# duylebkHCM/doc2tex

Hardware: AMD Instinct MI355X
Metric: formulas/s (greedy decode, 128x512 crops) (higher is better)
Workload: dtype bf16x3

## Files before the change

doc2tex_amd/_lib.py:

```python
import ctypes as C
import os

_HERE = os.path.dirname(os.path.abspath(__file__))
LIB_PATH = os.path.join(_HERE, "csrc", "libd2t.so")
if os.environ.get("D2T_PROBE_LIB"):
    LIB_PATH = os.path.abspath(os.environ["D2T_PROBE_LIB"])

D2T_OK = 0
D2T_EINVAL, D2T_ENOMEM, D2T_EHIP, D2T_ESTATE = 1, 2, 3, 4
ENC_RESNET, ENC_HYBRID_VIT, ENC_VGG_BILSTM, ENC_RESNET_BILSTM, ENC_VGG = 0, 1, 2, 3, 4
DEC_TFM, DEC_ATTN = 0, 1
ATTN_KEYS_ALL_INIT_MEAN, ATTN_KEYS_NOCLS_INIT_CLS, ATTN_KEYS_ALL_INIT_FIRST = 0, 1, 2
ACT_NONE, ACT_RELU, ACT_GELU = 0, 1, 2
CONV_FP32, CONV_BF16X3, CONV_FP16X2, CONV_MIXED = 0, 1, 2, 3
ATTN_CELL_LOCATION, ATTN_CELL_BAHDANAU = 0, 1
VIT_POS_SINCOS_PREFIX, VIT_POS_LEARNED_INTERP, VIT_POS_LEARNED_PREFIX = 0, 1, 2


class D2TConfig(C.Structure):
    _fields_ = [(n, C.c_int32) for n in (
        "encoder", "in_channels", "backbone_out", "vit_depth", "vit_heads", "vit_dim", "patch_h", "patch_w",
        "max_h", "max_w", "dec_dim", "dec_heads", "dec_layers", "dec_ff", "vocab", "max_seq_len",
        "decoder", "attn_hidden", "attn_kernel_size", "attn_kernel_dim", "attn_keys", "attn_enc_init",
        "attn_coverage", "bilstm_hidden", "batch_max_length", "gcb", "attn_cell", "attn_onehot", "vit_pos",
        "proj_height")]


class D2TPrepConfig(C.Structure):
    _fields_ = [(n, C.c_int32) for n in ("max_h", "max_w", "min_h", "min_w", "downsample", "variant")] + \
               [("mean", C.c_float), ("std", C.c_float), ("norm_mode", C.c_int32), ("channels", C.c_int32)]


class D2TPrepPlan(C.Structure):
    _fields_ = [(n, C.c_int32) for n in ("src_h", "src_w", "ds_h", "ds_w", "rs_h", "rs_w", "out_h", "out_w",
                                         "min_branch", "status")]


class D2TOpAttnDecodeArgs(C.Structure):
    _fields_ = [(n, C.c_void_p) for n in (
        "mem", "kp", "wq_t", "bq", "wloc", "bloc", "wscore", "wx_t", "bx", "wg_t", "bg", "wih_t", "bih", "wic_t", "bic", "emb",
        "tokgate", "probs", "tokens", "end_step", "st_h_in", "st_c_in", "st_mem_in", "st_h_out", "st_c_out", "st_mem_out",
        "tok_in", "row_sample", "teacher", "use_teacher", "out_dropmask", "sv_tok", "sv_hprev", "sv_cprev", "sv_hafter",
        "sv_cafter", "sv_gates", "sv_alpha", "sv_hq", "sv_x", "exit_state", "steps_dev")] + \
        [("bscore", C.c_float), ("out_dropscale", C.c_float)] + \
        [(n, C.c_int32) for n in ("B", "T", "S", "V", "taps", "key_off", "init_mode", "coverage", "end_token", "step_mode",
                                  "first", "samples")]
# ... 128 lines not shown
    "d2t_set_mixed_units": (_I, [_P, _I]),
    "d2t_set_reserved_blocks": (_I, [_P, _I]),
    "d2t_set_decode_chains": (_I, [_P, _I]),
    "d2t_set_conv_kernel": (_I, [_P, _I]),
    "d2t_set_conv_fusion": (_I, [_P, _I, _I]),
    "d2t_set_beam_shared_tile": (_I, [_P, _I]),
    "d2t_set_reserved_cus": (_I, [_P, _I]),
    "d2t_train_forward": (_I, [_P, _P, _I, _I, _I, _P, _I, _P, _P]),
    "d2t_train_backward": (_I, [_P, _P, _P]),
    "d2t_train_grad": (_I, [_P, C.c_char_p, _P, C.c_int64, _P]),
    "d2t_reload_weights": (_I, [_P, _I, C.POINTER(C.c_char_p), C.POINTER(C.c_void_p), C.POINTER(C.c_int64), _P]),
    "d2t_train_gather": (_I, [_P, _I, _I, C.POINTER(C.c_char_p), C.POINTER(C.c_int64), C.POINTER(C.c_int64), _P, _P]),
    "d2t_read_weight": (_I, [_P, C.c_char_p, _P, C.c_int64, _P]),
    "d2t_train_set_dropout": (_I, [_P, C.c_float, C.c_uint64]),
    "d2t_train_set_teacher_flags": (_I, [_P, C.c_char_p, _I]),
    "d2t_train_mask_count": (_I, [_P]),
    "d2t_train_decision_count": (_I, [_P]),
    "d2t_train_read_decision": (_I, [_P, _I, _P, C.c_int64, C.POINTER(_I), C.POINTER(C.c_int64), _P]),
    "d2t_train_read_mask": (_I, [_P, _I, _P, C.c_int64, _P]),
    "d2t_train_read_attn_alpha": (_I, [_P, _P, C.c_int64, _P]),
    "d2t_train_release": (None, [_P]),
    "d2t_profile_enable": (_I, [_P, _I]),
    "d2t_profile_read": (_I, [_P, _I, C.POINTER(_I)] + [C.POINTER(_I)] * 3 + [C.POINTER(C.c_float)]),
    "d2t_op_conv2d": (_I, [_P] * 5 + [_I] * 12 + [_P]),
    "d2t_op_conv2d_bf16x3": (_I, [_P] * 5 + [_I] * 12 + [_P]),
    "d2t_op_conv2d_bf16x3_split": (_I, [_P] * 5 + [_I] * 12 + [_P]),
    "d2t_op_conv2d_bf16x3_split_pool": (_I, [_P] * 4 + [_I] * 12 + [_P]),
    "d2t_op_set_conv_kernel": (_I, [_I, _I]),
    "d2t_op_linear": (_I, [_P] * 5 + [_I] * 4 + [_P]),
    "d2t_op_maxpool2x2": (_I, [_P, _P] + [_I] * 8 + [_P]),
    "d2t_op_layernorm": (_I, [_P] * 4 + [_I, _I, C.c_float, _P]),
    "d2t_op_vit_attention": (_I, [_P, _P, _I, _I, _I, _P]),
    "d2t_op_vit_attention_probs": (_I, [_P, _P, _P, _I, _I, _I, _P]),
    "d2t_op_decode_attention": (_I, [_P] * 4 + [_I] * 5 + [_P]),
    "d2t_op_skinny": (_I, [_P] * 6 + [C.c_float, _P, _P] + [_I] * 6 + [_P, _L, _P]),
    "d2t_op_skinny_form": (_I, [_P] * 6 + [C.c_float, _P, _P] + [_I] * 6 + [_P, _L, _I, _P]),
    "d2t_op_decoder_row": (_I, [_I] + [_P] * 13 + [C.c_float, _P, _P] + [_I] * 7 + [_P, _P, _I, _P, _I, _P]),
    "d2t_op_decoder_row_ragged": (_I, [_I] + [_P] * 13 + [C.c_float, _P, _P] + [_I] * 4 + [C.POINTER(_I), C.POINTER(_I), _P]),
    "d2t_op_decoder_row_ragged_beam": (_I, [_I] + [_P] * 13 + [C.c_float, _P, _P] + [_I] * 5 +
                                       [C.POINTER(_I), C.POINTER(_I), _P, _P, _I, _P]),
    "d2t_op_cross_attn_probs": (_I, [_P, _P, _I, _I, _I, _I, _P, _P]),
    "d2t_op_argmax_embed": (_I, [_P, _I] + [_P] * 13 + [_I] * 6 + [_P]),
    "d2t_op_beam_topk": (_I, [_P, _P, _P] + [_I] * 4 + [_P, _P, _P]),
    "d2t_op_beam_advance": (_I, [_I, _L] + [_P] * 15 + [_I] * 6 + [_P]),
    "d2t_op_beam_ancestry": (_I, [_P, _P, _P, _I, _I, _P, _P, _P, _P, _P]),
    "d2t_op_cache_gather": (_I, [_P, _P, _P] + [_I] * 7 + [_P]),
    "d2t_op_records_split": (_I, [_P, _P, _L, _I, _I, _P]),
    "d2t_op_records_merge": (_I, [_P, _P, _L, _I, _I, _P]),
    "d2t_op_conv_records": (_I, [C.POINTER(D2TOpConvRecordsArgs), _P]),
    "d2t_op_linear_kv": (_I, [_P] * 4 + [_I] * 7 + [_P]),
    "d2t_op_maxpool_records": (_I, [_P, _P] + [_I] * 9 + [_P]),
    "d2t_op_stem_records": (_I, [_P] * 4 + [_I] * 6 + [_P]),
    "d2t_op_pack_conv": (_I, [_P] * 6 + [C.c_float] + [_P] * 6 + [_I] * 4 + [_P]),
    "d2t_ce_forward": (_I, [_P, _P, _P, _P, _I, _I, _L, _P]),
    "d2t_ce_backward": (_I, [_P, _P, _P, _P, _P, _I, _I, _L, _P]),
    "d2t_ce_smooth_forward": (_I, [_P] * 6 + [_I, _I, _L, C.c_float, C.c_float, _I, _L, _P]),
    "d2t_ce_smooth_backward": (_I, [_P] * 7 + [_I, _I, _L, C.c_float, C.c_float, _I, _L, _P]),
    "d2t_optim_create": (_I, [C.POINTER(_P)]),
    "d2t_optim_destroy": (None, [_P]),
    "d2t_optim_last_error": (C.c_char_p, [_P]),
    "d2t_optim_chunk": (_I, []),
    "d2t_optim_step": (_I, [_P, C.POINTER(D2TOptimTensor), _I, _I, C.c_float, _P, _P]),
    "d2t_optim_lamb_step": (_I, [_P, C.POINTER(D2TOptimLambTensor), _I, C.c_float, _P, _P]),
    "d2t_optim_adamp_step": (_I, [_P, C.POINTER(D2TOptimAdampTensor), _I, C.c_float, _P, _P]),
    "d2t_optim_madgrad_step": (_I, [_P, C.POINTER(D2TOptimMadgradTensor), _I, C.c_float, _P, _P]),
    "d2t_optim_lookahead_sync": (_I, [_P, C.POINTER(D2TOptimLookaheadTensor), _I, C.c_float, _P]),
# ... 114 lines not shown
```

doc2tex_amd/csrc/engine.hip:

```cpp
#include "engine_impl.h"
#include <mutex>

#pragma clang diagnostic ignored "-Wc++20-designator"

namespace {

void vgg_hw(int H, int W, int* oh, int* ow) {
  *oh = H / 2 / 2 / 2 / 2 - 1;
  *ow = W / 2 / 2 - 1;
}
bool vgg_encoder(const d2t_config& g) { return g.encoder == D2T_ENC_VGG_BILSTM || g.encoder == D2T_ENC_VGG; }
bool lstm_encoder(const d2t_config& g) { return g.encoder == D2T_ENC_VGG_BILSTM || g.encoder == D2T_ENC_RESNET_BILSTM; }

int proj_height_check(d2t_ctx* c, int fh) {
  if (fh == 3) return D2T_OK;
  return fail(c, D2T_EINVAL, "mean_height False: proj_feat reads a feature map of height 3 (64-pixel crops), this crop gives "
              "height %d", fh);
}

void backbone_hw(int H, int W, int* oh, int* ow) {
  int h = H / 2, w = W / 2;
  h /= 2; w /= 2;
  h = (h - 2) / 2 + 1; w = w + 1;
  h = (h - 2) / 2 + 1; w = w + 1;
// ... 325 lines not shown
}

int patch_embed(d2t_ctx* c, hipStream_t s, const Act& f, int gh, int gw, int dim, float* X) {
  const d2t_config& g = c->cfg;
  const int T = gh * gw + 1;
  ConvP p{};
  p.out = X;
  if (int rc = conv_operands(c, s, p, c->patch, f)) return rc;
  conv_shape(p, f.B, f.H, f.W, f.C, dim, g.patch_h, g.patch_w, g.patch_h, g.patch_w, 0, 0, gh, gw);
  const float* pos;
  if (int rc = pos_table_for(c, gh, gw, s, &pos)) return rc;
  p.row_add = pos; p.rows_per_img = gh * gw; p.img_stride = T; p.row_off = 1; p.row_add_off = 1;
  HIPCHK(c, conv_timed(c, p, s));
  HIPCHK(c, launch_fill_cls(c->cls_row, X, f.B, (long long)T * dim, dim, s));
  return D2T_OK;
}

int encode_vit(d2t_ctx* c, hipStream_t s, const float* image, int B, int H, int W, int gh, int gw, int dim, float* memory,
               float* const* maps_dev, int n_maps) {
  Act f{};
  if (int rc = run_backbone(c, s, image, B, H, W, &f, nullptr, nullptr, true)) return rc;
  const Net n{c, s};
  float* X = n.pick({f.p});
  if (int rc = patch_embed(c, s, f, gh, gw, dim, X)) return rc;
  const int T = gh * gw + 1, M = B * T;
  float* Hn = n.pick({X});
  float* Q = n.pick({X, Hn});
  float* X2 = n.pick({X, Hn, Q});
  for (size_t i = 0; i < c->vit.size(); ++i) {
    const VitBlock& vb = c->vit[i];
    HIPCHK(c, launch_layernorm(X, vb.n1.g, vb.n1.b, Hn, M, dim, 1e-6f, s));
    HIPCHK(c, linear_any(c, s, Hn, vb.qkv, nullptr, Q, M, ACT_NONE));
    float* map = i < (size_t)n_maps ? maps_dev[i] : nullptr;
    if (map) HIPCHK(c, launch_vit_attention_probs(Q, Hn, map, B, T, c->cfg.vit_heads, s));
    else HIPCHK(c, launch_vit_attention(Q, Hn, B, T, c->cfg.vit_heads, s));
    HIPCHK(c, linear_any(c, s, Hn, vb.proj, X, X2, M, ACT_NONE));
    HIPCHK(c, launch_layernorm(X2, vb.n2.g, vb.n2.b, Hn, M, dim, 1e-6f, s));
    HIPCHK(c, linear_any(c, s, Hn, vb.fc1, nullptr, Q, M, ACT_GELU));
    HIPCHK(c, linear_any(c, s, Q, vb.fc2, X2, X, M, ACT_NONE));
  }
  HIPCHK(c, launch_layernorm(X, c->vit_norm.g, c->vit_norm.b, memory, M, dim, 1e-6f, s));
  return D2T_OK;
}

}

int d2t_internal_pe2d(d2t_ctx* c, int h, int w, int C, hipStream_t s, const float** out) { return get_pe2d(c, h, w, C, s, out); }
hipError_t d2t_internal_conv_timed(d2t_ctx* c, const ConvP& p, hipStream_t s) { return conv_timed(c, p, s); }

namespace {
std::mutex g_stream_mu;
std::map<std::pair<int, int>, std::vector<hipStream_t>> g_stream_pool;
hipError_t acquire_stream(int device, int prio, hipStream_t* out) {
  {
    std::lock_guard<std::mutex> lk(g_stream_mu);
    auto& v = g_stream_pool[std::make_pair(device, prio)];
    if (!v.empty()) {
      *out = v.back();
      v.pop_back();
      return hipSuccess;
    }
  }
  return hipStreamCreateWithPriority(out, hipStreamNonBlocking, prio);
}
void release_stream(int device, int prio, hipStream_t st) {
  hipStreamSynchronize(st);
  std::lock_guard<std::mutex> lk(g_stream_mu);
  g_stream_pool[std::make_pair(device, prio)].push_back(st);
// ... 312 lines not shown
```

doc2tex_amd/csrc/engine_ops.hip:

```cpp
#include <climits>

#include "engine_impl.h"

extern "C" {

int d2t_op_conv2d(const float* x, const float* w, const float* bias, const float* residual, float* y, int32_t B,
                  int32_t H, int32_t W, int32_t Cin, int32_t Cout, int32_t KH, int32_t KW, int32_t SH, int32_t SW,
                  int32_t PH, int32_t PW, int32_t act, d2t_stream stream) {
  if (!x || !w || !y || SH < 1 || SW < 1) return D2T_EINVAL;
  hipStream_t s = (hipStream_t)stream;
  if (Cin == 1 || Cin == 3) {
    if (KH != 3 || KW != 3 || SH != 1 || SW != 1 || PH != 1 || PW != 1 || residual) return D2T_EINVAL;
    return launch_stem(x, w, bias, y, B, Cin, H, W, Cout, act, s) == hipSuccess ? D2T_OK : D2T_EHIP;
  }
  if (Cin % 32) return D2T_EINVAL;
  float* wp = nullptr;
  if (hipMalloc(reinterpret_cast<void**>(&wp), (size_t)Cout * KH * KW * Cin * 4) != hipSuccess) return D2T_ENOMEM;
  ConvP p{};
  p.in = x; p.w = wp; p.bias = bias; p.res = residual; p.out = y;
  conv_shape(p, B, H, W, Cin, Cout, KH, KW, SH, SW, PH, PW);
  p.act = act;
  hipError_t e = launch_repack_ohwi(w, wp, Cout, KH, KW, Cin, s);
  if (e == hipSuccess) e = launch_conv(p, s);
  hipStreamSynchronize(s);
// ... 253 lines not shown

int d2t_op_maxpool2x2(const float* x, float* y, int32_t B, int32_t H, int32_t W, int32_t C, int32_t SH, int32_t SW,
                      int32_t PH, int32_t PW, d2t_stream stream) {
  if (!x || !y) return D2T_EINVAL;
  return launch_maxpool(x, y, B, H, W, C, SH, SW, PH, PW, (hipStream_t)stream) == hipSuccess ? D2T_OK : D2T_EHIP;
}

int d2t_op_layernorm(const float* x, const float* gamma, const float* beta, float* y, int32_t rows, int32_t D,
                     float eps, d2t_stream stream) {
  if (!x || !gamma || !beta || !y) return D2T_EINVAL;
  return launch_layernorm(x, gamma, beta, y, rows, D, eps, (hipStream_t)stream) == hipSuccess ? D2T_OK : D2T_EHIP;
}

int d2t_op_global_context(float* x, const float* wg, const float* bg, const float* w1, const float* b1, const float* ln_g,
                          const float* ln_b, const float* w2, const float* b2, float* ctx_out, int32_t B, int32_t HW, int32_t C,
                          d2t_stream stream) {
  if (!x || !wg || !bg || !w1 || !b1 || !ln_g || !ln_b || !w2 || !b2) return D2T_EINVAL;
  if (B < 1 || B > 65535 || HW < 1 || HW > (1 << 24) || C < 4 || C > 512 || C % 4) return D2T_EINVAL;
  hipStream_t s = (hipStream_t)stream;
  const size_t nl = (size_t)B * HW, nc = (size_t)B * C;
  float* buf = nullptr;
  if (hipMalloc(reinterpret_cast<void**>(&buf), (nl + 2 * nc) * 4) != hipSuccess) return D2T_ENOMEM;
  float *logits = buf, *ctx = buf + nl, *y = ctx + nc;
  const GCParams w{wg, bg, w1, b1, ln_g, ln_b, w2, b2};
  hipError_t e = launch_global_context(x, w, logits, ctx, y, B, HW, C, s);
  if (e == hipSuccess && ctx_out) e = hipMemcpyAsync(ctx_out, ctx, nc * 4, hipMemcpyDeviceToDevice, s);
  hipStreamSynchronize(s);
  hipFree(buf);
  return op_status(e);
}

int d2t_op_vit_attention(const float* qkv, float* y, int32_t B, int32_t N, int32_t heads, d2t_stream stream) {
  if (!qkv || !y) return D2T_EINVAL;
  return launch_vit_attention(qkv, y, B, N, heads, (hipStream_t)stream) == hipSuccess ? D2T_OK : D2T_EHIP;
}

int d2t_op_vit_attention_probs(const float* qkv, float* y, float* probs, int32_t B, int32_t N, int32_t heads,
                               d2t_stream stream) {
  if (!qkv || !y || !probs || B < 1 || N < 1 || heads < 1) return D2T_EINVAL;
  return launch_vit_attention_probs(qkv, y, probs, B, N, heads, (hipStream_t)stream) == hipSuccess ? D2T_OK : D2T_EHIP;
}

int d2t_op_decode_attention(const float* q, const float* k, const float* v, float* y, int32_t B, int32_t heads,
                            int32_t hd, int32_t L, int32_t Lmax, d2t_stream stream) {
  if (!q || !k || !v || !y || L > Lmax) return D2T_EINVAL;
  DecAttnP p{};
  p.q = q; p.q_stride = heads * hd; p.k = const_cast<float*>(k); p.v = const_cast<float*>(v);
  p.y = y; p.y_stride = heads * hd; p.B = B; p.heads = heads; p.hd = hd; p.Lmax = Lmax; p.L = L;
  p.kv_batch_stride = (long long)heads * Lmax * hd;
  return launch_decode_attention(p, (hipStream_t)stream) == hipSuccess ? D2T_OK : D2T_EHIP;
}

namespace {
bool fetch_ints(hipStream_t s, const int* dev, size_t n, std::vector<int>* out) {
  out->resize(n);
  if (hipStreamSynchronize(s) != hipSuccess) return false;
  return n == 0 || hipMemcpy(out->data(), dev, n * sizeof(int), hipMemcpyDeviceToHost) == hipSuccess;
}
}

namespace {
int op_skinny(const float* x, const float* w, const float* bias, const float* res, const float* ln_g, const float* ln_b,
              float ln_eps, float* y, float* ln_out, int32_t M, int32_t K, int32_t N, int32_t ldx, int32_t ldy, int32_t act,
              const int32_t* step, int64_t out_step_stride, int form, d2t_stream stream) {
  if (!x || !w || !y || M < 1 || M > 65535 * 16 || N < 1 || K < 16 || K % 16 || ldx < K || ldx % 4 || ldy < N) return D2T_EINVAL;
  if (act != ACT_NONE && act != ACT_RELU && act != ACT_GELU) return D2T_EINVAL;
  if ((ln_g == nullptr) != (ln_b == nullptr) || (ln_out && !ln_g)) return D2T_EINVAL;
  hipStream_t s = (hipStream_t)stream;
  if (step) {
    std::vector<int> t;
    if (out_step_stride < 0 || !fetch_ints(s, step, 1, &t) || t[0] < 0) return D2T_EINVAL;
  }
  SkinnyP p{};
// ... 630 lines not shown
```

doc2tex_amd/csrc/kernels.h:

```cpp
#pragma once
#include <hip/hip_runtime.h>
#include <stdint.h>

#pragma GCC visibility push(hidden)
#include "attn_beam_host.h"
#pragma GCC visibility pop

#include <cstdlib>
#ifdef D2T_PROBES
#define D2T_PROBE_ENV(name) (getenv(name) ? atoi(getenv(name)) : 0)
#define D2T_PROBE_ENV_STR(name) getenv(name)
#else
#define D2T_PROBE_ENV(name) 0
#define D2T_PROBE_ENV_STR(name) (static_cast<const char*>(nullptr))
#endif

namespace d2t {

inline dim3 grid_1d(size_t n, size_t cap) { return dim3((unsigned)((n + 255) / 256 < cap ? (n + 255) / 256 : cap)); }

enum { ACT_NONE = 0, ACT_RELU = 1, ACT_GELU = 2 };
enum { STORE_ROWS = 0, STORE_KV = 1 };

struct ConvP {
// ... 118 lines not shown
hipError_t launch_attn_decode_finalize(const unsigned long long* exit_state, int* steps_dev, int B, int S, int V, int Tk,
                                       int64_t* tokens, float* probs, float* alpha, hipStream_t s);
hipError_t launch_attn_decode_finalize_group(const unsigned long long* exit_state, int* steps_dev, const int* row_batch,
                                             const int* batch_rows, int batches, int B, int S, int V, int64_t* tokens,
                                             float* probs, hipStream_t s);
struct AttnTrainBwdP {
  const float* dlogits;
  const float* mem; int T, D, key_off;
  const float* kp;
  const float *wg_t, *wih_raw, *whh_raw, *wq_raw, *wloc, *bloc, *wscore;
  int taps;
  const float *sv_cprev, *sv_cafter, *sv_gates, *sv_alpha, *sv_hq;
  float* dmem;
  float* dkp;
  float *dgates, *dhq, *demb;
  const float* dhl = nullptr;
  float *dh0, *dc0;
  float *dwloc, *dbloc, *dwscore, *dbscore;
  int B, S, V, H, E, coverage;
  int probe = 0;
};
hipError_t launch_attn_train_lstm_bwd(const AttnTrainBwdP& p, hipStream_t s);
hipError_t launch_loc_unfold_bwd(const float* dwloc, const float* dbloc, int B, const float* conv_w, const float* conv_b,
                                 const float* proj_w, int H, int kd, int taps, float* d_conv_w, float* d_conv_b,
                                 float* d_proj_w, float* d_proj_b, hipStream_t s);
hipError_t launch_sum_over_rows(const float* part, float* out, int B, int C, hipStream_t s);
hipError_t launch_gather_rows(const float* src, float* dst, const int* idx, int rows, int width, hipStream_t s);
hipError_t launch_attn_decode(const AttnDecP& p, hipStream_t s);
hipError_t launch_attn_alpha_gather(const float* hist, const int* path, const int* len, float* out, int N, int S, int cap,
                                    int Tk, hipStream_t s);
hipError_t launch_transpose_into(const float* src, int rows, int cols, float* dst, int ld, int row_off, hipStream_t s);
hipError_t launch_layernorm(const float* x, const float* g, const float* b, float* y, int rows, int D, float eps,
                            hipStream_t s);
hipError_t launch_vit_attention(const float* qkv, float* y, int B, int N, int heads, hipStream_t s);
hipError_t launch_vit_attention_probs(const float* qkv, float* y, float* maps, int B, int N, int heads, hipStream_t s);

struct DecAttnP {
  const float* q; int q_stride;
  float* k; float* v;
  long long kv_batch_stride;
  const float* cur_k; const float* cur_v; int cur_stride;
  float* y; int y_stride;
  int B, heads, hd, Lmax;
  int L;
  const int* step_ptr;
};
hipError_t launch_decode_attention(const DecAttnP& p, hipStream_t s);

struct DecRowP {
  const float* qkv; int qkv_stride;
  const float* xres;
  float* sk; float* sv; long long s_batch_stride; int s_Lmax;
  const float* ck; const float* cv; long long c_batch_stride; int T;
  const int* c_row_map;
  const float* wo_t; const float* bo;
  const float* ln1_g; const float* ln1_b; float eps;
  const float* wq_t; const float* bq;
  const float* wco_t; const float* bco;
  float* y2;
  const int* step_ptr;
  int M, D, heads;
  unsigned long long* trace;
  const int* stop_at;
  int probe;
  const int* anc; int anc_stride; int one_row;
  const int* rows_ptr;
};
hipError_t launch_decoder_row(const DecRowP& p, hipStream_t s);
// ... 221 lines not shown
```

doc2tex_amd/csrc/vit_attn.hip:

```cpp
#include "conv_common.h"

namespace d2t {


__device__ __forceinline__ int acc_row(int e, int h) { return (e & 3) + 8 * (e >> 2) + 4 * h; }

template <bool WITH_V>
__device__ __forceinline__ void stage_keys(float* Ks, float* Vs, const float* head, int C, int N, int t0, int Np, int tid,
                                           int nthreads) {
  for (int i = tid; i < Np * 8; i += nthreads) {
    const int jl = i >> 3, j = t0 * 32 + jl, c = (i & 7) * 4;
    float4 kv = make_float4(0.f, 0.f, 0.f, 0.f), vv = kv;
    if (j < N) {
      kv = *reinterpret_cast<const float4*>(head + (size_t)j * 3 * C + c);
      if (WITH_V) vv = *reinterpret_cast<const float4*>(head + (size_t)j * 3 * C + C + c);
    }
    float* kd = Ks + jl * 33 + c;
    kd[0] = kv.x; kd[1] = kv.y; kd[2] = kv.z; kd[3] = kv.w;
    if (WITH_V) *reinterpret_cast<float4*>(Vs + jl * 32 + c) = vv;
  }
}

__device__ __forceinline__ f32x16 score_tile(const float* Ks, int tl, int r, int h, const float (&qb)[16]) {
  f32x16 sacc;
#pragma unroll
  for (int e = 0; e < 16; ++e) sacc[e] = 0.f;
  const float* ka = Ks + (size_t)(tl * 32 + r) * 33 + h;
#pragma unroll
  for (int kk = 0; kk < 16; ++kk) sacc = __builtin_amdgcn_mfma_f32_32x32x2f32(ka[2 * kk], qb[kk], sacc, 0, 0, 0);
  return sacc;
}

template <bool MAPS>
__global__ __launch_bounds__(1024) void vit_attention_mfma_kernel(const float* __restrict__ qkv, float* __restrict__ y,
                                                                  float* __restrict__ maps, int N, int heads, int tiles,
                                                                  int kct, int qchunks) {
  extern __shared__ __attribute__((aligned(16))) float sm[];
  const int Np = kct * 32;
  float* Ks = sm;
  float* Vs = Ks + (size_t)Np * 33;
  const int bh = blockIdx.x / qchunks, qc = blockIdx.x % qchunks;
  const int b = bh / heads, hh = bh % heads, C = heads * 32;
  const float* base = qkv + (size_t)b * N * 3 * C;
  const float* khead = base + C + hh * 32;
  const int tid = threadIdx.x, wave = tid >> 6, lane = tid & 63, nthreads = blockDim.x;
  const int r = lane & 31, h = lane >> 5, q0 = (qc * 16 + wave) * 32;
  float qb[16];
  {
    const int row = q0 + r < N ? q0 + r : N - 1;
    const float* qp = base + (size_t)row * 3 * C + hh * 32;
    const float scale = 0.17677669529663687f;
#pragma unroll
    for (int kk = 0; kk < 16; ++kk) qb[kk] = qp[2 * kk + h] * scale;
  }
  f32x16 o;
#pragma unroll
  for (int e = 0; e < 16; ++e) o[e] = 0.f;
  float mrun = -INFINITY, lrun = 0.f;
  for (int t0 = 0; t0 < tiles; t0 += kct) {
    if (t0) __syncthreads();
    stage_keys<true>(Ks, Vs, khead, C, N, t0, Np, tid, nthreads);
    __syncthreads();
    const int tend = t0 + kct < tiles ? t0 + kct : tiles;
    for (int t = t0; t < tend; ++t) {
      const int tl = t - t0;
      const f32x16 sacc = score_tile(Ks, tl, r, h, qb);
      float sv[16], mx = -INFINITY;
#pragma unroll
      for (int e = 0; e < 16; ++e) {
        sv[e] = t * 32 + acc_row(e, h) < N ? sacc[e] : -INFINITY;
        mx = fmaxf(mx, sv[e]);
      }
      mx = fmaxf(mx, __shfl_xor(mx, 32, 64));
      const float mnew = fmaxf(mrun, mx);
      const float corr = expf(mrun - mnew);
      float pe[16], ps = 0.f;
#pragma unroll
      for (int e = 0; e < 16; ++e) {
        pe[e] = expf(sv[e] - mnew);
        ps += pe[e];
      }
      lrun = lrun * corr + ps;
      mrun = mnew;
#pragma unroll
      for (int e = 0; e < 16; ++e) o[e] *= __shfl(corr, acc_row(e, h), 64);
      const float* vb = Vs + (size_t)(tl * 32 + 4 * h) * 32 + r;
#pragma unroll
      for (int kk = 0; kk < 16; ++kk)
        o = __builtin_amdgcn_mfma_f32_32x32x2f32(pe[kk], vb[(size_t)acc_row(kk, 0) * 32], o, 0, 0, 0);
    }
  }
  lrun += __shfl_xor(lrun, 32, 64);
#pragma unroll
  for (int e = 0; e < 16; ++e) {
    const int qi = acc_row(e, h);
    const float l = __shfl(lrun, qi, 64);
    const int row = q0 + qi;
    if (row < N) y[((size_t)b * N + row) * C + hh * 32 + r] = o[e] / l;
  }
  if constexpr (MAPS) {
    __syncthreads();
    float* ws = Vs + (size_t)wave * 512;
    float* pm = maps + (size_t)bh * N * N;
    const int c = lane & 15;
    for (int t0 = 0; t0 < tiles; t0 += kct) {
      if (kct < tiles) {
        if (t0) __syncthreads();
        stage_keys<false>(Ks, nullptr, khead, C, N, t0, Np, tid, nthreads);
        __syncthreads();
      }
      const int tend = t0 + kct < tiles ? t0 + kct : tiles;
      for (int t = t0; t < tend; ++t) {
        const f32x16 sacc = score_tile(Ks, t - t0, r, h, qb);
#pragma unroll
        for (int half = 0; half < 2; ++half) {
#pragma unroll
          for (int i = 0; i < 8; ++i)
            ws[r * 16 + (acc_row(i, h) ^ ((r >> 1) & 15))] = expf(sacc[8 * half + i] - mrun) / lrun;
          __builtin_amdgcn_wave_barrier();
          __builtin_amdgcn_s_waitcnt(0xC07F);
          const int key = t * 32 + 16 * half + c;
#pragma unroll
          for (int i = 0; i < 8; ++i) {
            const int qr = 4 * i + (lane >> 4), row = q0 + qr;
            const float p = ws[qr * 16 + (c ^ ((qr >> 1) & 15))];
            if (row < N && key < N) pm[(size_t)row * N + key] = p;
          }
          __builtin_amdgcn_wave_barrier();
        }
      }
    }
  }
}

template <bool MAPS>
static hipError_t launch_vit_attention_mfma(const float* qkv, float* y, float* maps, int B, int N, int heads, hipStream_t s) {
  const int tiles = (N + 31) / 32;
  const int kct = tiles <= 16 ? tiles : 8, qchunks = (tiles + 15) / 16, waves = tiles < 16 ? tiles : 16;
  const size_t lds = ((size_t)kct * 32 * 33 + (size_t)kct * 32 * 32) * sizeof(float);
  static_assert(16 * 32 * (33 + 32) * sizeof(float) <= 160 * 1024, "the largest chunk (kct = 16) fits the CU's LDS");
  static bool attr_set = false;
  if (!attr_set) {
    hipError_t e = hipFuncSetAttribute(reinterpret_cast<const void*>(vit_attention_mfma_kernel<MAPS>),
                                       hipFuncAttributeMaxDynamicSharedMemorySize, 160 * 1024);
    if (e != hipSuccess) return e;
    attr_set = true;
  }
  hipLaunchKernelGGL(vit_attention_mfma_kernel<MAPS>, dim3(B * heads * qchunks), dim3(waves * 64), lds, s, qkv, y, maps, N,
                     heads, tiles, kct, qchunks);
  return hipGetLastError();
}

hipError_t launch_vit_attention(const float* qkv, float* y, int B, int N, int heads, hipStream_t s) {
  return launch_vit_attention_mfma<false>(qkv, y, nullptr, B, N, heads, s);
}

hipError_t launch_vit_attention_probs(const float* qkv, float* y, float* maps, int B, int N, int heads, hipStream_t s) {
  if (!maps) return launch_vit_attention(qkv, y, B, N, heads, s);
  return launch_vit_attention_mfma<true>(qkv, y, maps, B, N, heads, s);
}

}
```

include/d2t.h:

```cpp
#ifndef D2T_H
#define D2T_H

#include <stdint.h>

#ifdef __cplusplus
extern "C" {
#endif

typedef struct d2t_ctx d2t_ctx;
typedef void* d2t_stream;

enum {
  D2T_OK = 0,
  D2T_EINVAL = 1,
  D2T_ENOMEM = 2,
  D2T_EHIP = 3,
  D2T_ESTATE = 4
};

enum {
  D2T_ENC_RESNET = 0,
  D2T_ENC_HYBRID_VIT = 1,
  D2T_ENC_VGG_BILSTM = 2,
  D2T_ENC_RESNET_BILSTM = 3,
// ... 153 lines not shown
int d2t_train_mask_count(d2t_ctx* ctx);
int d2t_train_decision_count(d2t_ctx* ctx);
int d2t_train_read_decision(d2t_ctx* ctx, int32_t index, uint8_t* dst, int64_t numel, int32_t* is_pool_out,
                            int64_t* numel_out, d2t_stream stream);
int d2t_train_read_mask(d2t_ctx* ctx, int32_t index, uint8_t* dst, int64_t numel, d2t_stream stream);
int d2t_train_read_attn_alpha(d2t_ctx* ctx, float* dst, int64_t numel, d2t_stream stream);
void d2t_train_release(d2t_ctx* ctx);

int d2t_profile_enable(d2t_ctx* ctx, int32_t on);
int d2t_profile_read(d2t_ctx* ctx, int32_t max_records, int32_t* n, int32_t* M, int32_t* N, int32_t* K, float* ms);

int d2t_op_conv2d(const float* x, const float* w, const float* bias, const float* residual, float* y, int32_t B,
                  int32_t H, int32_t W, int32_t Cin, int32_t Cout, int32_t KH, int32_t KW, int32_t SH, int32_t SW,
                  int32_t PH, int32_t PW, int32_t act, d2t_stream stream);
int d2t_op_conv2d_bf16x3(const float* x, const float* w, const float* bias, const float* residual, float* y, int32_t B,
                         int32_t H, int32_t W, int32_t Cin, int32_t Cout, int32_t KH, int32_t KW, int32_t SH,
                         int32_t SW, int32_t PH, int32_t PW, int32_t act, d2t_stream stream);
int d2t_op_set_conv_kernel(int32_t kind, int32_t reserved_cus);
int d2t_op_conv2d_bf16x3_split_pool(const float* x, const float* w, const float* bias, float* y, int32_t B, int32_t H, int32_t W,
                                    int32_t Cin, int32_t Cout, int32_t KH, int32_t KW, int32_t SH, int32_t SW, int32_t PH,
                                    int32_t PW, int32_t act, d2t_stream stream);
int d2t_op_conv2d_bf16x3_split(const float* x, const float* w, const float* bias, const float* residual, float* y,
                               int32_t B, int32_t H, int32_t W, int32_t Cin, int32_t Cout, int32_t KH, int32_t KW,
                               int32_t SH, int32_t SW, int32_t PH, int32_t PW, int32_t act, d2t_stream stream);
int d2t_op_linear(const float* x, const float* w, const float* bias, const float* residual, float* y, int32_t M,
                  int32_t K, int32_t N, int32_t act, d2t_stream stream);
int d2t_op_maxpool2x2(const float* x, float* y, int32_t B, int32_t H, int32_t W, int32_t C, int32_t SH, int32_t SW,
                      int32_t PH, int32_t PW, d2t_stream stream);
int d2t_op_layernorm(const float* x, const float* gamma, const float* beta, float* y, int32_t rows, int32_t D,
                     float eps, d2t_stream stream);
int d2t_op_vit_attention(const float* qkv, float* y, int32_t B, int32_t N, int32_t heads, d2t_stream stream);
int d2t_op_vit_attention_probs(const float* qkv, float* y, float* probs, int32_t B, int32_t N, int32_t heads,
                               d2t_stream stream);
int d2t_op_decode_attention(const float* q, const float* k, const float* v, float* y, int32_t B, int32_t heads,
                            int32_t hd, int32_t L, int32_t Lmax, d2t_stream stream);

int d2t_op_skinny(const float* x, const float* w, const float* bias, const float* res, const float* ln_g, const float* ln_b,
                  float ln_eps, float* y, float* ln_out, int32_t M, int32_t K, int32_t N, int32_t ldx, int32_t ldy, int32_t act,
                  const int32_t* step, int64_t out_step_stride, d2t_stream stream);
int d2t_op_skinny_form(const float* x, const float* w, const float* bias, const float* res, const float* ln_g,
                       const float* ln_b, float ln_eps, float* y, float* ln_out, int32_t M, int32_t K, int32_t N, int32_t ldx,
                       int32_t ldy, int32_t act, const int32_t* step, int64_t out_step_stride, int32_t form,
                       d2t_stream stream);
int d2t_op_decoder_row(int32_t kind, const float* qkv, const float* xres, float* sk, float* sv, const float* mem,
                       const float* ca_in_w, const float* ca_in_b, const float* sa_out_w, const float* sa_out_b,
                       const float* ca_out_w, const float* ca_out_b, const float* ln1_g, const float* ln1_b, float eps, float* y2,
                       const int32_t* step, int32_t M, int32_t D, int32_t T, int32_t Lmax, int32_t rows, int32_t samples,
                       int32_t one_row, const int32_t* row_map, const int32_t* anc, int32_t anc_stride, const int32_t* seg,
                       int32_t nsamples, d2t_stream stream);
int d2t_op_decoder_row_ragged(int32_t kind, const float* qkv, const float* xres, float* sk, float* sv, const float* mem,
                              const float* ca_in_w, const float* ca_in_b, const float* sa_out_w, const float* sa_out_b,
                              const float* ca_out_w, const float* ca_out_b, const float* ln1_g, const float* ln1_b, float eps,
                              float* y2, const int32_t* step, int32_t M, int32_t Lmax, int32_t rows, int32_t mem_rows,
                              const int32_t* row0, const int32_t* len, d2t_stream stream);
int d2t_op_decoder_row_ragged_beam(int32_t kind, const float* qkv, const float* xres, float* sk, float* sv, const float* mem,
                                   const float* ca_in_w, const float* ca_in_b, const float* sa_out_w, const float* sa_out_b,
                                   const float* ca_out_w, const float* ca_out_b, const float* ln1_g, const float* ln1_b, float eps,
                                   float* y2, const int32_t* step, int32_t M, int32_t Lmax, int32_t rows, int32_t mem_rows,
                                   int32_t samples, const int32_t* row0, const int32_t* len, const int32_t* row_map,
                                   const int32_t* anc, int32_t anc_stride, d2t_stream stream);
int d2t_op_cross_attn_probs(const float* q, const float* keys, int32_t M, int32_t D, int32_t T, int32_t per_head, float* out,
                            d2t_stream stream);
int d2t_op_argmax_embed(const float* logits, int32_t S, int64_t* tokens, int32_t* ended, int32_t* end_count, int32_t* steps_done,
                        int32_t* step, int32_t* done_count, int32_t* batch_end_count, int32_t* batch_steps_done,
                        int32_t* batches_done, int32_t* stop_at, const float* emb, const float* pe, float* x, int32_t B, int32_t V,
                        int32_t d, int32_t end_token, int32_t rows_per_batch, int32_t n_batches, d2t_stream stream);
// ... 275 lines not shown
```

Before: 1615.

## Add bf16x3 split-precision path for ViT attention MFMA kernel

Adds a bf16x3 variant of the ViT flash-attention kernel. It splits Q, K, V and the probabilities into hi/lo bf16 planes in swizzled LDS, uses bf16 MFMA products instead of fp32 32x32x2 MFMA, reads V with transposing LDS loads, and uses exp2 with a log2e-folded scale. The path is selected when the bf16x3 conv mode is on and sequence length exceeds 32. It aims to replace the slow fp32 MFMA rate with faster bf16 MFMAs while keeping near-fp32 accuracy, at the cost of extra split arithmetic and a different LDS layout.

```diff
diff --git a/doc2tex_amd/_lib.py b/doc2tex_amd/_lib.py
--- a/doc2tex_amd/_lib.py
+++ b/doc2tex_amd/_lib.py
@@ -12,6 +12,7 @@
 DEC_TFM, DEC_ATTN = 0, 1
 ATTN_KEYS_ALL_INIT_MEAN, ATTN_KEYS_NOCLS_INIT_CLS, ATTN_KEYS_ALL_INIT_FIRST = 0, 1, 2
 ACT_NONE, ACT_RELU, ACT_GELU = 0, 1, 2
+VIT_ATTN_FP32, VIT_ATTN_BF16X3 = 0, 1
 CONV_FP32, CONV_BF16X3, CONV_FP16X2, CONV_MIXED = 0, 1, 2, 3
 ATTN_CELL_LOCATION, ATTN_CELL_BAHDANAU = 0, 1
 VIT_POS_SINCOS_PREFIX, VIT_POS_LEARNED_INTERP, VIT_POS_LEARNED_PREFIX = 0, 1, 2
@@ -206,6 +207,7 @@
     "d2t_op_layernorm": (_I, [_P] * 4 + [_I, _I, C.c_float, _P]),
     "d2t_op_vit_attention": (_I, [_P, _P, _I, _I, _I, _P]),
     "d2t_op_vit_attention_probs": (_I, [_P, _P, _P, _I, _I, _I, _P]),
+    "d2t_op_vit_attention_form": (_I, [_P, _P, _P, _I, _I, _I, _I, _P]),
     "d2t_op_decode_attention": (_I, [_P] * 4 + [_I] * 5 + [_P]),
     "d2t_op_skinny": (_I, [_P] * 6 + [C.c_float, _P, _P] + [_I] * 6 + [_P, _L, _P]),
     "d2t_op_skinny_form": (_I, [_P] * 6 + [C.c_float, _P, _P] + [_I] * 6 + [_P, _L, _I, _P]),
diff --git a/doc2tex_amd/csrc/engine.hip b/doc2tex_amd/csrc/engine.hip
--- a/doc2tex_amd/csrc/engine.hip
+++ b/doc2tex_amd/csrc/engine.hip
@@ -381,8 +381,7 @@
     HIPCHK(c, launch_layernorm(X, vb.n1.g, vb.n1.b, Hn, M, dim, 1e-6f, s));
     HIPCHK(c, linear_any(c, s, Hn, vb.qkv, nullptr, Q, M, ACT_NONE));
     float* map = i < (size_t)n_maps ? maps_dev[i] : nullptr;
-    if (map) HIPCHK(c, launch_vit_attention_probs(Q, Hn, map, B, T, c->cfg.vit_heads, s));
-    else HIPCHK(c, launch_vit_attention(Q, Hn, B, T, c->cfg.vit_heads, s));
+    HIPCHK(c, launch_vit_attention(Q, Hn, map, B, T, c->cfg.vit_heads, c->conv_bf16x3 && vit_attention_bx3_pays(T), s));
     HIPCHK(c, linear_any(c, s, Hn, vb.proj, X, X2, M, ACT_NONE));
     HIPCHK(c, launch_layernorm(X2, vb.n2.g, vb.n2.b, Hn, M, dim, 1e-6f, s));
     HIPCHK(c, linear_any(c, s, Hn, vb.fc1, nullptr, Q, M, ACT_GELU));
diff --git a/doc2tex_amd/csrc/engine_ops.hip b/doc2tex_amd/csrc/engine_ops.hip
--- a/doc2tex_amd/csrc/engine_ops.hip
+++ b/doc2tex_amd/csrc/engine_ops.hip
@@ -309,13 +309,20 @@
 
 int d2t_op_vit_attention(const float* qkv, float* y, int32_t B, int32_t N, int32_t heads, d2t_stream stream) {
   if (!qkv || !y) return D2T_EINVAL;
-  return launch_vit_attention(qkv, y, B, N, heads, (hipStream_t)stream) == hipSuccess ? D2T_OK : D2T_EHIP;
+  return launch_vit_attention(qkv, y, nullptr, B, N, heads, false, (hipStream_t)stream) == hipSuccess ? D2T_OK : D2T_EHIP;
 }
 
 int d2t_op_vit_attention_probs(const float* qkv, float* y, float* probs, int32_t B, int32_t N, int32_t heads,
                                d2t_stream stream) {
   if (!qkv || !y || !probs || B < 1 || N < 1 || heads < 1) return D2T_EINVAL;
-  return launch_vit_attention_probs(qkv, y, probs, B, N, heads, (hipStream_t)stream) == hipSuccess ? D2T_OK : D2T_EHIP;
+  return launch_vit_attention(qkv, y, probs, B, N, heads, false, (hipStream_t)stream) == hipSuccess ? D2T_OK : D2T_EHIP;
+}
+
+int d2t_op_vit_attention_form(const float* qkv, float* y, float* probs, int32_t B, int32_t N, int32_t heads, int32_t form,
+                              d2t_stream stream) {
+  if (!qkv || !y || B < 1 || N < 1 || heads < 1 || (form != D2T_VIT_ATTN_FP32 && form != D2T_VIT_ATTN_BF16X3)) return D2T_EINVAL;
+  return launch_vit_attention(qkv, y, probs, B, N, heads, form == D2T_VIT_ATTN_BF16X3, (hipStream_t)stream) == hipSuccess
+             ? D2T_OK : D2T_EHIP;
 }
 
 int d2t_op_decode_attention(const float* q, const float* k, const float* v, float* y, int32_t B, int32_t heads,
diff --git a/doc2tex_amd/csrc/kernels.h b/doc2tex_amd/csrc/kernels.h
--- a/doc2tex_amd/csrc/kernels.h
+++ b/doc2tex_amd/csrc/kernels.h
@@ -174,8 +174,8 @@
 hipError_t launch_transpose_into(const float* src, int rows, int cols, float* dst, int ld, int row_off, hipStream_t s);
 hipError_t launch_layernorm(const float* x, const float* g, const float* b, float* y, int rows, int D, float eps,
                             hipStream_t s);
-hipError_t launch_vit_attention(const float* qkv, float* y, int B, int N, int heads, hipStream_t s);
-hipError_t launch_vit_attention_probs(const float* qkv, float* y, float* maps, int B, int N, int heads, hipStream_t s);
+hipError_t launch_vit_attention(const float* qkv, float* y, float* maps, int B, int N, int heads, bool bx3, hipStream_t s);
+inline bool vit_attention_bx3_pays(int N) { return N > 32; }
 
 struct DecAttnP {
   const float* q; int q_stride;
diff --git a/doc2tex_amd/csrc/vit_attn.hip b/doc2tex_amd/csrc/vit_attn.hip
--- a/doc2tex_amd/csrc/vit_attn.hip
+++ b/doc2tex_amd/csrc/vit_attn.hip
@@ -5,53 +5,163 @@
 
 __device__ __forceinline__ int acc_row(int e, int h) { return (e & 3) + 8 * (e >> 2) + 4 * h; }
 
-template <bool WITH_V>
-__device__ __forceinline__ void stage_keys(float* Ks, float* Vs, const float* head, int C, int N, int t0, int Np, int tid,
+typedef __bf16 bf16x4 __attribute__((ext_vector_type(4)));
+typedef short s16x4 __attribute__((ext_vector_type(4)));
+typedef short s16x8 __attribute__((ext_vector_type(8)));
+typedef __attribute__((address_space(3))) s16x4* lds_s16x4_ptr;
+
+__device__ __forceinline__ void split_rne(float x, __bf16& hi, __bf16& lo) {
+  hi = (__bf16)x;
+  lo = (__bf16)(x - (float)hi);
+}
+__device__ __forceinline__ void split_rne4(const float4& v, bf16x4& hi, bf16x4& lo) {
+  __bf16 h, l;
+  split_rne(v.x, h, l); hi[0] = h; lo[0] = l;
+  split_rne(v.y, h, l); hi[1] = h; lo[1] = l;
+  split_rne(v.z, h, l); hi[2] = h; lo[2] = l;
+  split_rne(v.w, h, l); hi[3] = h; lo[3] = l;
+}
+
+template <bool BX3>
+struct KeyChunk {
+  unsigned char* base;
+  int Np;
+  __device__ __forceinline__ size_t v_off() const { return BX3 ? (size_t)Np * 2 * XROW : (size_t)Np * 33 * sizeof(float); }
+  __device__ __forceinline__ float* Ks() const { return reinterpret_cast<float*>(base); }
+  __device__ __forceinline__ float* Vs() const { return reinterpret_cast<float*>(base + v_off()); }
+  __device__ __forceinline__ unsigned char* plane(int i) const { return base + (size_t)i * Np * XROW; }
+};
+
+template <bool WITH_V, bool BX3>
+__device__ __forceinline__ void stage_keys(const KeyChunk<BX3>& kc, const float* head, int C, int N, int t0, int tid,
                                            int nthreads) {
-  for (int i = tid; i < Np * 8; i += nthreads) {
+  for (int i = tid; i < kc.Np * 8; i += nthreads) {
     const int jl = i >> 3, j = t0 * 32 + jl, c = (i & 7) * 4;
     float4 kv = make_float4(0.f, 0.f, 0.f, 0.f), vv = kv;
     if (j < N) {
       kv = *reinterpret_cast<const float4*>(head + (size_t)j * 3 * C + c);
       if (WITH_V) vv = *reinterpret_cast<const float4*>(head + (size_t)j * 3 * C + C + c);
     }
-    float* kd = Ks + jl * 33 + c;
-    kd[0] = kv.x; kd[1] = kv.y; kd[2] = kv.z; kd[3] = kv.w;
-    if (WITH_V) *reinterpret_cast<float4*>(Vs + jl * 32 + c) = vv;
-  }
-}
-
-__device__ __forceinline__ f32x16 score_tile(const float* Ks, int tl, int r, int h, const float (&qb)[16]) {
+    if constexpr (BX3) {
+      const int off = jl * XROW + swz_chunk(jl, c >> 3) * 16 + (c & 4) * 2;
+      bf16x4 hi, lo;
+      split_rne4(kv, hi, lo);
+      *reinterpret_cast<bf16x4*>(kc.plane(0) + off) = hi;
+      *reinterpret_cast<bf16x4*>(kc.plane(1) + off) = lo;
+      if (WITH_V) {
+        split_rne4(vv, hi, lo);
+        *reinterpret_cast<bf16x4*>(kc.plane(2) + off) = hi;
+        *reinterpret_cast<bf16x4*>(kc.plane(3) + off) = lo;
+      }
+    } else {
+      float* kd = kc.Ks() + jl * 33 + c;
+      kd[0] = kv.x; kd[1] = kv.y; kd[2] = kv.z; kd[3] = kv.w;
+      if (WITH_V) *reinterpret_cast<float4*>(kc.Vs() + jl * 32 + c) = vv;
+    }
+  }
+}
+
+template <bool BX3>
+__device__ __forceinline__ float softmax_exp(float x) {
+  if constexpr (BX3) return __builtin_amdgcn_exp2f(x);
+  else return expf(x);
+}
+template <bool BX3>
+constexpr float Q_SCALE = BX3 ? 0.25503348668941584f : 0.17677669529663687f;
+
+template <bool BX3>
+struct QOperand {
+  float f[16];
+  __device__ __forceinline__ void load(const float* qp, int h, float scale) {
+#pragma unroll
+    for (int kk = 0; kk < 16; ++kk) f[kk] = qp[2 * kk + h] * scale;
+  }
+};
+template <>
+struct QOperand<true> {
+  bf16x8 hi[2], lo[2];
+  __device__ __forceinline__ void load(const float* qp, int h, float scale) {
+#pragma unroll
+    for (int ks = 0; ks < 2; ++ks)
+#pragma unroll
+      for (int i = 0; i < 8; ++i) {
+        __bf16 a, b;
+        split_rne(qp[16 * ks + 8 * h + i] * scale, a, b);
+        hi[ks][i] = a; lo[ks][i] = b;
+      }
+  }
+};
+
+template <bool BX3>
+__device__ __forceinline__ f32x16 score_tile(const KeyChunk<BX3>& kc, int tl, int r, int h, const QOperand<BX3>& q) {
   f32x16 sacc;
 #pragma unroll
   for (int e = 0; e < 16; ++e) sacc[e] = 0.f;
-  const float* ka = Ks + (size_t)(tl * 32 + r) * 33 + h;
-#pragma unroll
-  for (int kk = 0; kk < 16; ++kk) sacc = __builtin_amdgcn_mfma_f32_32x32x2f32(ka[2 * kk], qb[kk], sacc, 0, 0, 0);
+  if constexpr (BX3) {
+#pragma unroll
+    for (int ks = 0; ks < 2; ++ks) {
+      bf16x8 kh[1], kl[1];
+      read_frags32(kc.plane(0), kc.plane(1), tl * 32 + r, 2 * ks + h, kh, kl);
+      sacc = product(sacc, kh[0], kl[0], q.hi[ks], q.lo[ks]);
+    }
+  } else {
+    const float* ka = kc.Ks() + (size_t)(tl * 32 + r) * 33 + h;
+#pragma unroll
+    for (int kk = 0; kk < 16; ++kk) sacc = __builtin_amdgcn_mfma_f32_32x32x2f32(ka[2 * kk], q.f[kk], sacc, 0, 0, 0);
+  }
   return sacc;
 }
 
-template <bool MAPS>
-__global__ __launch_bounds__(1024) void vit_attention_mfma_kernel(const float* __restrict__ qkv, float* __restrict__ y,
-                                                                  float* __restrict__ maps, int N, int heads, int tiles,
-                                                                  int kct, int qchunks) {
-  extern __shared__ __attribute__((aligned(16))) float sm[];
-  const int Np = kct * 32;
-  float* Ks = sm;
-  float* Vs = Ks + (size_t)Np * 33;
+template <bool BX3>
+__device__ __forceinline__ f32x16 weighted_sum(f32x16 o, const KeyChunk<BX3>& kc, int tl, int lane, const float (&pe)[16]) {
+  const int r = lane & 31, h = lane >> 5;
+  if constexpr (BX3) {
+    const int l16 = lane & 15, col = 16 * ((lane >> 4) & 1) + 4 * (l16 & 3);
+#pragma unroll
+    for (int ks = 0; ks < 2; ++ks) {
+      bf16x8 ph, pl;
+#pragma unroll
+      for (int i = 0; i < 8; ++i) {
+        __bf16 a, b;
+        split_rne(pe[8 * ks + i], a, b);
+        ph[i] = a; pl[i] = b;
+      }
+      const int j0 = tl * 32 + 16 * ks + 4 * h + (l16 >> 2), j1 = j0 + 8;
+      const int off0 = j0 * XROW + swz_chunk(j0, col >> 3) * 16 + (col & 4) * 2;
+      const int off1 = j1 * XROW + swz_chunk(j1, col >> 3) * 16 + (col & 4) * 2;
+      const s16x4 h0 = __builtin_amdgcn_ds_read_tr16_b64_v4i16((lds_s16x4_ptr)(kc.plane(2) + off0));
+      const s16x4 h1 = __builtin_amdgcn_ds_read_tr16_b64_v4i16((lds_s16x4_ptr)(kc.plane(2) + off1));
+      const s16x4 l0 = __builtin_amdgcn_ds_read_tr16_b64_v4i16((lds_s16x4_ptr)(kc.plane(3) + off0));
+      const s16x4 l1 = __builtin_amdgcn_ds_read_tr16_b64_v4i16((lds_s16x4_ptr)(kc.plane(3) + off1));
+      const s16x8 vh = {h0[0], h0[1], h0[2], h0[3], h1[0], h1[1], h1[2], h1[3]};
+      const s16x8 vl = {l0[0], l0[1], l0[2], l0[3], l1[0], l1[1], l1[2], l1[3]};
+      o = product(o, __builtin_bit_cast(bf16x8, vh), __builtin_bit_cast(bf16x8, vl), ph, pl);
+    }
+  } else {
+    const float* vb = kc.Vs() + (size_t)(tl * 32 + 4 * h) * 32 + r;
+#pragma unroll
+    for (int kk = 0; kk < 16; ++kk)
+      o = __builtin_amdgcn_mfma_f32_32x32x2f32(pe[kk], vb[(size_t)acc_row(kk, 0) * 32], o, 0, 0, 0);
+  }
+  return o;
+}
+
+template <bool MAPS, bool BX3>
+__global__ __launch_bounds__(1024) __attribute__((amdgpu_waves_per_eu(5)))
+void vit_attention_mfma_kernel(const float* __restrict__ qkv, float* __restrict__ y, float* __restrict__ maps, int N, int heads,
+                               int tiles, int kct, int qchunks) {
+  extern __shared__ __attribute__((aligned(16))) unsigned char sm[];
+  const KeyChunk<BX3> kc{sm, kct * 32};
   const int bh = blockIdx.x / qchunks, qc = blockIdx.x % qchunks;
   const int b = bh / heads, hh = bh % heads, C = heads * 32;
   const float* base = qkv + (size_t)b * N * 3 * C;
   const float* khead = base + C + hh * 32;
   const int tid = threadIdx.x, wave = tid >> 6, lane = tid & 63, nthreads = blockDim.x;
   const int r = lane & 31, h = lane >> 5, q0 = (qc * 16 + wave) * 32;
-  float qb[16];
+  QOperand<BX3> qb;
   {
     const int row = q0 + r < N ? q0 + r : N - 1;
-    const float* qp = base + (size_t)row * 3 * C + hh * 32;
-    const float scale = 0.17677669529663687f;
-#pragma unroll
-    for (int kk = 0; kk < 16; ++kk) qb[kk] = qp[2 * kk + h] * scale;
+    qb.load(base + (size_t)row * 3 * C + hh * 32, h, Q_SCALE<BX3>);
   }
   f32x16 o;
 #pragma unroll
@@ -59,70 +169,87 @@
   float mrun = -INFINITY, lrun = 0.f;
   for (int t0 = 0; t0 < tiles; t0 += kct) {
     if (t0) __syncthreads();
-    stage_keys<true>(Ks, Vs, khead, C, N, t0, Np, tid, nthreads);
+    stage_keys<true>(kc, khead, C, N, t0, tid, nthreads);
     __syncthreads();
     const int tend = t0 + kct < tiles ? t0 + kct : tiles;
     for (int t = t0; t < tend; ++t) {
       const int tl = t - t0;
-      const f32x16 sacc = score_tile(Ks, tl, r, h, qb);
+      const f32x16 sacc = score_tile(kc, tl, r, h, qb);
       float sv[16], mx = -INFINITY;
-#pragma unroll
-      for (int e = 0; e < 16; ++e) {
-        sv[e] = t * 32 + acc_row(e, h) < N ? sacc[e] : -INFINITY;
-        mx = fmaxf(mx, sv[e]);
-      }
+      if (BX3 && t != tiles - 1) {
+#pragma unroll
+        for (int e = 0; e < 16; ++e) sv[e] = sacc[e];
+      } else {
+#pragma unroll
+        for (int e = 0; e < 16; ++e) sv[e] = t * 32 + acc_row(e, h) < N ? sacc[e] : -INFINITY;
+      }
+#pragma unroll
+      for (int e = 0; e < 16; ++e) mx = fmaxf(mx, sv[e]);
       mx = fmaxf(mx, __shfl_xor(mx, 32, 64));
       const float mnew = fmaxf(mrun, mx);
-      const float corr = expf(mrun - mnew);
+      const float corr = softmax_exp<BX3>(mrun - mnew);
       float pe[16], ps = 0.f;
 #pragma unroll
       for (int e = 0; e < 16; ++e) {
-        pe[e] = expf(sv[e] - mnew);
+        pe[e] = softmax_exp<BX3>(sv[e] - mnew);
         ps += pe[e];
       }
       lrun = lrun * corr + ps;
       mrun = mnew;
-#pragma unroll
-      for (int e = 0; e < 16; ++e) o[e] *= __shfl(corr, acc_row(e, h), 64);
-      const float* vb = Vs + (size_t)(tl * 32 + 4 * h) * 32 + r;
-#pragma unroll
-      for (int kk = 0; kk < 16; ++kk)
-        o = __builtin_amdgcn_mfma_f32_32x32x2f32(pe[kk], vb[(size_t)acc_row(kk, 0) * 32], o, 0, 0, 0);
+      if constexpr (BX3) {
+#pragma unroll
+        for (int e = 0; e < 16; ++e) o[e] *= corr;
+      } else {
+#pragma unroll
+        for (int e = 0; e < 16; ++e) o[e] *= __shfl(corr, acc_row(e, h), 64);
+      }
+      o = weighted_sum(o, kc, tl, lane, pe);
     }
   }
   lrun += __shfl_xor(lrun, 32, 64);
-#pragma unroll
-  for (int e = 0; e < 16; ++e) {
-    const int qi = acc_row(e, h);
-    const float l = __shfl(lrun, qi, 64);
-    const int row = q0 + qi;
-    if (row < N) y[((size_t)b * N + row) * C + hh * 32 + r] = o[e] / l;
+  const int le = __lane_id(), re = le & 31, he = le >> 5;
+  if constexpr (BX3) {
+    if (q0 + re < N) {
+      float* yr = y + ((size_t)b * N + q0 + re) * C + hh * 32 + 4 * he;
+#pragma unroll
+      for (int g = 0; g < 4; ++g)
+        *reinterpret_cast<float4*>(yr + 8 * g) =
+            make_float4(o[4 * g] / lrun, o[4 * g + 1] / lrun, o[4 * g + 2] / lrun, o[4 * g + 3] / lrun);
+    }
+  } else {
+#pragma unroll
+    for (int e = 0; e < 16; ++e) {
+      const int qi = acc_row(e, he);
+      const float l = __shfl(lrun, qi, 64);
+      const int row = q0 + qi;
+      if (row < N) y[((size_t)b * N + row) * C + hh * 32 + re] = o[e] / l;
+    }
   }
   if constexpr (MAPS) {
     __syncthreads();
-    float* ws = Vs + (size_t)wave * 512;
+    float* ws = kc.Vs() + (size_t)wave * 512;
     float* pm = maps + (size_t)bh * N * N;
-    const int c = lane & 15;
+    const int c = le & 15;
     for (int t0 = 0; t0 < tiles; t0 += kct) {
       if (kct < tiles) {
         if (t0) __syncthreads();
-        stage_keys<false>(Ks, nullptr, khead, C, N, t0, Np, tid, nthreads);
+        stage_keys<false>(kc, khead, C, N, t0, tid, nthreads);
         __syncthreads();
       }
       const int tend = t0 + kct < tiles ? t0 + kct : tiles;
       for (int t = t0; t < tend; ++t) {
-        const f32x16 sacc = score_tile(Ks, t - t0, r, h, qb);
+        const f32x16 sacc = score_tile(kc, t - t0, re, he, qb);
 #pragma unroll
         for (int half = 0; half < 2; ++half) {
 #pragma unroll
           for (int i = 0; i < 8; ++i)
-            ws[r * 16 + (acc_row(i, h) ^ ((r >> 1) & 15))] = expf(sacc[8 * half + i] - mrun) / lrun;
+            ws[re * 16 + (acc_row(i, he) ^ ((re >> 1) & 15))] = softmax_exp<BX3>(sacc[8 * half + i] - mrun) / lrun;
           __builtin_amdgcn_wave_barrier();
           __builtin_amdgcn_s_waitcnt(0xC07F);
           const int key = t * 32 + 16 * half + c;
 #pragma unroll
           for (int i = 0; i < 8; ++i) {
-            const int qr = 4 * i + (lane >> 4), row = q0 + qr;
+            const int qr = 4 * i + (le >> 4), row = q0 + qr;
             const float p = ws[qr * 16 + (c ^ ((qr >> 1) & 15))];
             if (row < N && key < N) pm[(size_t)row * N + key] = p;
           }
@@ -133,31 +260,30 @@
   }
 }
 
-template <bool MAPS>
+template <bool MAPS, bool BX3>
 static hipError_t launch_vit_attention_mfma(const float* qkv, float* y, float* maps, int B, int N, int heads, hipStream_t s) {
   const int tiles = (N + 31) / 32;
   const int kct = tiles <= 16 ? tiles : 8, qchunks = (tiles + 15) / 16, waves = tiles < 16 ? tiles : 16;
-  const size_t lds = ((size_t)kct * 32 * 33 + (size_t)kct * 32 * 32) * sizeof(float);
+  const size_t lds = (size_t)kct * 32 * (BX3 ? 4 * XROW : (33 + 32) * sizeof(float));
   static_assert(16 * 32 * (33 + 32) * sizeof(float) <= 160 * 1024, "the largest chunk (kct = 16) fits the CU's LDS");
+  static_assert(8 * 32 * 128 >= 16 * 512 * sizeof(float), "a chunked launch's V half holds sixteen waves' map scratch");
   static bool attr_set = false;
   if (!attr_set) {
-    hipError_t e = hipFuncSetAttribute(reinterpret_cast<const void*>(vit_attention_mfma_kernel<MAPS>),
+    hipError_t e = hipFuncSetAttribute(reinterpret_cast<const void*>(vit_attention_mfma_kernel<MAPS, BX3>),
                                        hipFuncAttributeMaxDynamicSharedMemorySize, 160 * 1024);
     if (e != hipSuccess) return e;
     attr_set = true;
   }
-  hipLaunchKernelGGL(vit_attention_mfma_kernel<MAPS>, dim3(B * heads * qchunks), dim3(waves * 64), lds, s, qkv, y, maps, N,
-                     heads, tiles, kct, qchunks);
+  hipLaunchKernelGGL((vit_attention_mfma_kernel<MAPS, BX3>), dim3(B * heads * qchunks), dim3(waves * 64), lds, s, qkv, y, maps,
+                     N, heads, tiles, kct, qchunks);
   return hipGetLastError();
 }
 
-hipError_t launch_vit_attention(const float* qkv, float* y, int B, int N, int heads, hipStream_t s) {
-  return launch_vit_attention_mfma<false>(qkv, y, nullptr, B, N, heads, s);
-}
-
-hipError_t launch_vit_attention_probs(const float* qkv, float* y, float* maps, int B, int N, int heads, hipStream_t s) {
-  if (!maps) return launch_vit_attention(qkv, y, B, N, heads, s);
-  return launch_vit_attention_mfma<true>(qkv, y, maps, B, N, heads, s);
-}
-
-}
+hipError_t launch_vit_attention(const float* qkv, float* y, float* maps, int B, int N, int heads, bool bx3, hipStream_t s) {
+  if (bx3) return maps ? launch_vit_attention_mfma<true, true>(qkv, y, maps, B, N, heads, s)
+                       : launch_vit_attention_mfma<false, true>(qkv, y, nullptr, B, N, heads, s);
+  return maps ? launch_vit_attention_mfma<true, false>(qkv, y, maps, B, N, heads, s)
+              : launch_vit_attention_mfma<false, false>(qkv, y, nullptr, B, N, heads, s);
+}
+
+}
diff --git a/include/d2t.h b/include/d2t.h
--- a/include/d2t.h
+++ b/include/d2t.h
@@ -209,6 +209,10 @@
 int d2t_op_vit_attention(const float* qkv, float* y, int32_t B, int32_t N, int32_t heads, d2t_stream stream);
 int d2t_op_vit_attention_probs(const float* qkv, float* y, float* probs, int32_t B, int32_t N, int32_t heads,
                                d2t_stream stream);
+#define D2T_VIT_ATTN_FP32 0
+#define D2T_VIT_ATTN_BF16X3 1
+int d2t_op_vit_attention_form(const float* qkv, float* y, float* probs, int32_t B, int32_t N, int32_t heads, int32_t form,
+                              d2t_stream stream);
 int d2t_op_decode_attention(const float* q, const float* k, const float* v, float* y, int32_t B, int32_t heads,
                             int32_t hd, int32_t L, int32_t Lmax, d2t_stream stream);
 
```

Result: faster. 1632, median of 6 (+1.1%).
